# trvon/yams

Hardware: AMD Instinct MI355X
Metric: k-NN QPS + recall@k, 100M x 768 fp32 cosine top-100; ingest GB/s SHA-256+CDC (higher is better)
Workload: dtype i8 (MFMA filter, exact i32 accumulate) + f64 (exact re-score)

## Files before the change

### yams_amd/csrc/scan_i8_kernel.hip

```cpp
#include <cstdlib>
#include <type_traits>

#include "lds_dma.h"
#include "scan_args.h"

namespace yams_accel {

using i32x4v = __attribute__((ext_vector_type(4))) int;

constexpr int I8_ROWS = 256, I8_QUERIES = 256, I8_THREADS = 512;
constexpr int I8_SLAB = 64;
constexpr int I8_NST = 4;
constexpr int I8_A_BYTES = I8_ROWS * I8_SLAB;
constexpr int I8_B_BYTES = I8_QUERIES * I8_SLAB;
constexpr int I8_STAGE = I8_A_BYTES + I8_B_BYTES;
constexpr int I8_BLOCK_ROWS = 64;

__device__ __forceinline__ int i8_swz(int row) {
    const int j = (row >> 2) & 3;
    return (((j ^ (j >> 1)) & 1) << 1) | (j >> 1);
}

__host__ __device__ __forceinline__ uint64_t i8_blocked_offset(uint64_t row, uint32_t col, uint32_t dim) {
    const uint32_t j = static_cast<uint32_t>(row & 15u), slab = col >> 6, chunk = (col >> 4) & 3u;
// ... 1586 lines not shown
    const double per_wave = 8192.0 * p.tau_rank * p.sample_stride / static_cast<double>(p.n_rows ? p.n_rows : 1) * (L.i8_l2 ? 2.0 : 1.0);
    const uint32_t c = static_cast<uint32_t>(per_wave * 4.0 < 8192.0 ? per_wave * 4.0 : 8192.0) + 16;
    return (c + 15) / 16 * 16 < 8192u ? (c + 15) / 16 * 16 : 8192u;
}

hipError_t launch_i8_log_gather(hipStream_t st, const ScanLaunch& L) {
    const uint64_t regions = i8_log_regions(L);
    if (regions == 0) return hipSuccess;
    const ResidentPlan rp = i8_resident_plan(L);
    const I8GatherL2 l2{L.i8_l2_meta, L.i8_row_bias, L.i8_q_bias, L.rows_nsq, L.tau, L.l2_eps};
#ifdef YAMS_ACCEL_MEASURE
    if (rp.use && L.i8_q_form) {
        hipLaunchKernelGGL(i8_log_gather_blocks_kernel, dim3(static_cast<uint32_t>(regions)), dim3(256), 0, st,
                           reinterpret_cast<const int32_t*>(L.log_key), L.log_cnt, L.log_cap, rp.n_qt, L.rows_i8_meta, L.q_meta, L.q_thr,
                           L.plan.n_rows, L.row_mask, L.list_count, L.list, L.plan.list_cap);
        return hipGetLastError();
    }
#endif
    if (rp.use) {
        if (L.i8_l2)
            hipLaunchKernelGGL((i8_log_gather_wave_kernel<true>), dim3(static_cast<uint32_t>(regions)), dim3(256), 0, st,
                               L.log_key, L.log_q, L.log_cnt, L.log_cap, rp.n_qt, L.rows_i8_meta, L.q_meta, L.q_thr, L.list_count,
                               L.list, L.plan.list_cap, l2);
        else
            hipLaunchKernelGGL((i8_log_gather_wave_kernel<false>), dim3(static_cast<uint32_t>(regions)), dim3(256), 0, st,
                               L.log_key, L.log_q, L.log_cnt, L.log_cap, rp.n_qt, L.rows_i8_meta, L.q_meta, L.q_thr, L.list_count,
                               L.list, L.plan.list_cap, l2);
        return hipGetLastError();
    }
    if (L.i8_l2)
        hipLaunchKernelGGL((i8_log_gather_kernel<true>), dim3(static_cast<uint32_t>((regions + 255) / 256)), dim3(256), 0, st,
                           L.log_key, L.log_q, L.log_cnt, L.log_cap, regions, L.rows_i8_meta, L.q_meta, L.q_thr, L.list_count, L.list,
                           L.plan.list_cap, l2);
    else
        hipLaunchKernelGGL((i8_log_gather_kernel<false>), dim3(static_cast<uint32_t>((regions + 255) / 256)), dim3(256), 0, st,
                           L.log_key, L.log_q, L.log_cnt, L.log_cap, regions, L.rows_i8_meta, L.q_meta, L.q_thr, L.list_count, L.list,
                           L.plan.list_cap, l2);
    return hipGetLastError();
}

static bool i8r_direct_rows(uint32_t dim, uint32_t n_qt, bool l2) { (void)dim; return l2 ? n_qt >= 4 : true; }

hipError_t launch_scan_i8(hipStream_t st, const ScanLaunch& L, int mode, int version) {
    (void)version;
    ScanArgs a = make_scan_args(L);
    a.n_sel_tiles = mode == MODE_SAMPLE ? L.plan.n_sample_tiles : L.plan.n_filter_tiles;
    if (a.n_sel_tiles == 0) return hipSuccess;
    const uint32_t hgrid = ((2u * a.n_sel_tiles + 7) / 8) * a.n_qtiles * 8;
    const ResidentPlan rp = i8_resident_plan(L);
    if (mode == MODE_SAMPLE) {
        const uint32_t s_units = (L.plan.n_sample_tiles + 1u) / 2u;
        bool resident_sample = rp.use && !L.i8_l2 && L.i8_sync && L.plan.sample_stride >= 2 && !L.i8_sample_small_grid &&
                               (L.i8_form == 2 ? s_units >= 1u : s_units >= 4u * rp.n_streams);
#ifdef YAMS_ACCEL_MEASURE
        if (const char* sv = std::getenv("YAMS_ACCEL_I8R_SAMPLE")) resident_sample = resident_sample && std::atoi(sv) != 0;
        if (version != 2 && version != 3 && version != 0) resident_sample = false;
#endif
        if (resident_sample) {
            a.i8_sync = L.i8_sync + i8_sync_words(L) / 2u;
            hipLaunchKernelGGL((scan_tiles_i8r_kernel<0, false, true, 0, true>), dim3(rp.grid), dim3(R_THREADS), 0, st, a, s_units, rp.n_qt, rp.n_streams, 1u);
        } else if (L.i8_l2) hipLaunchKernelGGL((scan_tiles_i8h_kernel<MODE_SAMPLE, 0, YAMS_SCAN_L2>), dim3(hgrid), dim3(H_THREADS), 0, st, a);
        else hipLaunchKernelGGL((scan_tiles_i8h_kernel<MODE_SAMPLE>), dim3(hgrid), dim3(H_THREADS), 0, st, a);
        return hipGetLastError();
    }
    bool direct = i8r_direct_rows(L.plan.dim, rp.n_qt, L.i8_l2);
#ifdef YAMS_ACCEL_MEASURE
    if (const char* dv = std::getenv("YAMS_ACCEL_I8R_DIRECT")) direct = std::atoi(dv) != 0;
#endif
    if (L.i8_l2) {
        a.rows_i8_meta = L.i8_l2_meta;
        uint32_t l2_pace_log2 = direct ? 2u : 0u;
#ifdef YAMS_ACCEL_MEASURE
        if (const char* pv = std::getenv("YAMS_ACCEL_I8R_L2_PACE_LOG2")) l2_pace_log2 = static_cast<uint32_t>(std::atoi(pv)) & 31u;
#endif
        const uint32_t l2_window = 1u | (l2_pace_log2 << 16);
        if (rp.use && direct) hipLaunchKernelGGL((scan_tiles_i8r_kernel<0, true, true>), dim3(rp.grid), dim3(R_THREADS), 0, st, a, rp.n_units, rp.n_qt, rp.n_streams, l2_window);
        else if (rp.use) hipLaunchKernelGGL((scan_tiles_i8r_kernel<0, true>), dim3(rp.grid), dim3(R_THREADS), 0, st, a, rp.n_units, rp.n_qt, rp.n_streams, 1u);
        else hipLaunchKernelGGL((scan_tiles_i8h_kernel<MODE_FILTER, 0, YAMS_SCAN_L2>), dim3(hgrid), dim3(H_THREADS), 0, st, a);
        return hipGetLastError();
    }
    uint32_t pace_log2 = direct ? 2u : 0u;
    uint32_t window = 1;
#ifdef YAMS_ACCEL_MEASURE
    if (version >= 41 && version <= 48) {
        if (version == 41) hipLaunchKernelGGL((scan_tiles_i8h_kernel<MODE_FILTER, 1>), dim3(hgrid), dim3(H_THREADS), 0, st, a);
        else if (version == 42) hipLaunchKernelGGL((scan_tiles_i8h_kernel<MODE_FILTER, 2>), dim3(hgrid), dim3(H_THREADS), 0, st, a);
        else if (version == 43) hipLaunchKernelGGL((scan_tiles_i8h_kernel<MODE_FILTER, 3>), dim3(hgrid), dim3(H_THREADS), 0, st, a);
        else if (version == 44) hipLaunchKernelGGL((scan_tiles_i8h_kernel<MODE_FILTER, 4>), dim3(hgrid), dim3(H_THREADS), 0, st, a);
        else if (version == 45) hipLaunchKernelGGL((scan_tiles_i8h_kernel<MODE_FILTER, 5>), dim3(hgrid), dim3(H_THREADS), 0, st, a);
        else if (version == 46) hipLaunchKernelGGL((scan_tiles_i8h_kernel<MODE_FILTER, 6>), dim3(hgrid), dim3(H_THREADS), 0, st, a);
        else if (version == 48) hipLaunchKernelGGL((scan_tiles_i8h_kernel<MODE_FILTER, 8>), dim3(hgrid), dim3(H_THREADS), 0, st, a);
        else hipLaunchKernelGGL((scan_tiles_i8h_kernel<MODE_FILTER, 7>), dim3(hgrid), dim3(H_THREADS), 0, st, a);
        return hipGetLastError();
    }
    if (const char* wv = std::getenv("YAMS_ACCEL_I8R_WINDOW")) window = static_cast<uint32_t>(std::atoi(wv)) & 0xffffu;
    if (const char* pv = std::getenv("YAMS_ACCEL_I8R_PACE_LOG2")) pace_log2 = static_cast<uint32_t>(std::atoi(pv)) & 31u;
    window |= pace_log2 << 16; pace_log2 = 0;
    if (rp.use && version >= 61 && version <= 69) {
        if (version == 61) hipLaunchKernelGGL((scan_tiles_i8r_kernel<1>), dim3(rp.grid), dim3(R_THREADS), 0, st, a, rp.n_units, rp.n_qt, rp.n_streams, window);
        else if (version == 62) hipLaunchKernelGGL((scan_tiles_i8r_kernel<2>), dim3(rp.grid), dim3(R_THREADS), 0, st, a, rp.n_units, rp.n_qt, rp.n_streams, window);
        else if (version == 64) hipLaunchKernelGGL((scan_tiles_i8r_kernel<4>), dim3(rp.grid), dim3(R_THREADS), 0, st, a, rp.n_units, rp.n_qt, rp.n_streams, window);
        else if (version == 68) hipLaunchKernelGGL((scan_tiles_i8r_kernel<8>), dim3(rp.grid), dim3(R_THREADS), 0, st, a, rp.n_units, rp.n_qt, rp.n_streams, window);
        else if (version == 66) hipLaunchKernelGGL((scan_tiles_i8r_kernel<9>), dim3(rp.grid), dim3(R_THREADS), 0, st, a, rp.n_units, rp.n_qt, rp.n_streams, window);
        else if (version == 69) hipLaunchKernelGGL((scan_tiles_i8r_kernel<10, false, true>), dim3(rp.grid), dim3(R_THREADS), 0, st, a, rp.n_units, rp.n_qt, rp.n_streams, window);
        else if (version == 65) hipLaunchKernelGGL((scan_tiles_i8r_kernel<7, false, true>), dim3(rp.grid), dim3(R_THREADS), 0, st, a, rp.n_units, rp.n_qt, rp.n_streams, window);
        else hipLaunchKernelGGL((scan_tiles_i8r_kernel<7>), dim3(rp.grid), dim3(R_THREADS), 0, st, a, rp.n_units, rp.n_qt, rp.n_streams, window);
        return hipGetLastError();
    }
    if (version == 40) {
        hipLaunchKernelGGL((scan_tiles_i8h_kernel<MODE_FILTER>), dim3(hgrid), dim3(H_THREADS), 0, st, a);
        return hipGetLastError();
    }
    if (rp.use && version == 90 && (L.plan.dim == 384 || L.plan.dim == 768)) {
// ... 42 lines not shown
```

### yams_amd/csrc/scan_i8d_kernel.h

```cpp
template <int DUMMY = 0>
__global__ __launch_bounds__(R_THREADS, 1) void scan_tiles_i8d_kernel(ScanArgs a, uint32_t n_units, uint32_t n_qt, uint32_t n_streams, uint32_t window) {
    const uint32_t pace_mask = (1u << ((window >> 16) & 255u)) - 1u;
    __shared__ __attribute__((aligned(16))) unsigned char lds[R_LDS];

    const uint32_t bid = blockIdx.x;
    const uint32_t xcd = bid & 7u, slot = bid >> 3;
    const uint32_t qt = slot % n_qt, st = slot / n_qt;
    if (st >= (n_streams >> 3)) return;
    const uint32_t stream = st * 8u + xcd;
    if (stream >= n_units) return;

#ifdef YAMS_ACCEL_MEASURE
    const uint64_t t_begin = wall_clock64();
#endif
    const int tid = threadIdx.x;
    const int lane = tid & 63;
    const int wid = __builtin_amdgcn_readfirstlane(tid >> 6);
    const int l15 = lane & 15, lq = lane >> 4;
    const uint32_t dim = a.dim;
    const int nslab = dim / I8_SLAB;
    const uint32_t q0 = qt * R_QUERIES;
    const uint32_t lds0 = static_cast<uint32_t>(reinterpret_cast<uintptr_t>((__attribute__((address_space(3))) unsigned char*)lds));
    const uint64_t n_blocks = (a.n_rows + I8_BLOCK_ROWS - 1) / I8_BLOCK_ROWS;
    const uint64_t past_end = n_blocks * I8_BLOCK_ROWS;
    const uint32_t piece_row_stride = static_cast<uint32_t>(nslab) * 1024u;

    struct Geo { uint64_t row0; const unsigned char* base; };
    auto unit_of = [&](uint32_t k) __attribute__((always_inline)) -> uint32_t { return stream + (k >> 1) * n_streams; };
    auto locate = [&](uint32_t k, Geo& g) __attribute__((always_inline)) {
        const uint32_t un_ = unit_of(k);
        const uint32_t sel = un_ < n_units ? 2u * un_ + (k & 1u) : 0xffffffffu;
        uint64_t row0 = past_end;
        if (sel < a.n_sel_tiles) {
            const uint32_t tile = sel + sel / (a.stride - 1u) + 1u;
            row0 = static_cast<uint64_t>(tile) * I8_ROWS + static_cast<uint32_t>((wid & 3) * 64);
        }
        g.row0 = row0;
        const uint64_t rowb = row0 < past_end ? row0 : past_end - 64;
        g.base = reinterpret_cast<const unsigned char*>(a.rows_i8) + (rowb / 16) * piece_row_stride;
    };
    typedef float f2_t __attribute__((ext_vector_type(2)));
    auto meta_ptr = [&](uint64_t row0) __attribute__((always_inline)) -> const float* {
        uint64_t blk = row0 / I8_BLOCK_ROWS;
        if (blk >= n_blocks) blk = n_blocks - 1;
        return a.rows_i8_meta + 2ull * blk;
    };

    {
        const int prow = lane >> 2;
        const int rowB = wid * 16 + prow;
        const uint32_t voffB = static_cast<uint32_t>(rowB) * 64u + ((lane & 3) ^ i8_swz(prow)) * 16u;
        const unsigned char* baseB = reinterpret_cast<const unsigned char*>(a.q_i8) + static_cast<uint64_t>(q0) * 64;
        const uint64_t qslab_bytes = static_cast<uint64_t>(a.q_pad) * 64;
        for (int s = 0; s < nslab; ++s)
            lds_dma16_s(baseB + s * qslab_bytes, voffB, __builtin_amdgcn_readfirstlane(lds0 + s * R_B_SLAB + wid * 1024));
    }
    if (tid < R_QUERIES) reinterpret_cast<f2_t*>(lds + R_ZS_THR)[tid] = reinterpret_cast<const f2_t*>(a.q_thr)[q0 + static_cast<uint32_t>(tid)];
    uint32_t* const pair_cnt = a.i8_sync + (static_cast<uint64_t>(stream) * 4u + static_cast<uint32_t>(wid & 3)) * 32u;
    uint32_t take_v;
    auto take_request = [&]() __attribute__((always_inline)) {
        unsigned long long keep;
        asm volatile("s_mov_b64 %1, exec\n\ts_mov_b64 exec, 1\n\tglobal_atomic_add %0, %2, %3, off sc0\n\ts_mov_b64 exec, %1"
                     : "=&v"(take_v), "=&s"(keep) : "v"(pair_cnt + qt), "v"(1u) : "memory");
    };
    auto take_result = [&]() __attribute__((always_inline)) -> uint32_t {
        asm volatile("" : "+v"(take_v));
        return static_cast<uint32_t>(__builtin_amdgcn_readfirstlane(static_cast<int>(take_v)));
    };
    uint32_t k_cur, k_nxt, k_fut;
    take_request(); asm volatile("s_waitcnt vmcnt(0)" ::: "memory"); k_cur = take_result();
    take_request(); asm volatile("s_waitcnt vmcnt(0)" ::: "memory"); k_nxt = take_result();
    take_request(); asm volatile("s_waitcnt vmcnt(0)" ::: "memory"); k_fut = take_result();
    Geo cur, nxt;
    locate(k_cur, cur);
    float sb, eb;
    {
        const float* mp = meta_ptr(cur.row0);
        const float m0 = mp[0], m1 = mp[1];
        sb = __int_as_float(__builtin_amdgcn_readfirstlane(__float_as_int(m0)));
        eb = __int_as_float(__builtin_amdgcn_readfirstlane(__float_as_int(m1)));
    }
    asm volatile("s_waitcnt vmcnt(0) lgkmcnt(0)" ::: "memory");
    __builtin_amdgcn_s_barrier();

    const int offF = l15 * 64 + ((lq ^ i8_swz(l15)) << 4);
    i32x4v acc[4][8];
    i32x4v fa[3][4], fb[4];
    auto dfetch = [](i32x4v& dst, uint32_t vo, const unsigned char* src) __attribute__((always_inline)) {
        asm volatile("global_load_dwordx4 %0, %1, %2" : "=v"(dst) : "v"(vo), "s"(src) : "memory");
    };
    auto ldq = [&](int slab, int cb) __attribute__((always_inline)) -> i32x4v {
        return *reinterpret_cast<const i32x4v*>(lds + slab * R_B_SLAB + offF + cb * 1024);
    };
#pragma unroll
    for (int rb = 0; rb < 4; ++rb) dfetch(fa[0][rb], static_cast<uint32_t>(offF), cur.base + static_cast<uint32_t>(rb) * piece_row_stride);
#pragma unroll
    for (int rb = 0; rb < 4; ++rb) dfetch(fa[1][rb], static_cast<uint32_t>(offF), cur.base + 1024u + static_cast<uint32_t>(rb) * piece_row_stride);
#pragma unroll
    for (int cb = 0; cb < 3; ++cb) fb[cb] = ldq(0, cb);

    constexpr uint32_t R_POLLS = 1024;
    bool pacing = true;
    const uint32_t R_WINDOW = window & 0xffffu;
    const uint32_t* sync_sib = pair_cnt + (static_cast<uint32_t>(lane) < n_qt ? static_cast<uint32_t>(lane) : qt);
#ifdef YAMS_ACCEL_MEASURE
    uint32_t units_read = 0;
#endif
    uint32_t q_live = 0;
#pragma unroll
    for (int cb = 0; cb < 8; ++cb) q_live |= (q0 + static_cast<uint32_t>(cb * 16 + l15) < a.n_queries) ? 1u << cb : 0u;

    const f2_t* const thr_lds = reinterpret_cast<const f2_t*>(lds + R_ZS_THR) + l15;
    auto acc_init = [&](float sb_, float eb_) __attribute__((always_inline)) {
        const float is = 1.0f / sb_, g = eb_ * is;
#pragma unroll
        for (int cb = 0; cb < 8; ++cb) {
            const f2_t h = thr_lds[cb * 16];
            const int nt = i8_neg_threshold(h[0], is, h[1], g);
#pragma unroll
            for (int rb = 0; rb < 4; ++rb)
#pragma unroll
                for (int r = 0; r < 4; ++r) acc[rb][cb][r] = nt;
        }
    };
    const uint32_t log_region = (stream * n_qt + qt) * 8u + static_cast<uint32_t>(wid);
    const uint64_t region = static_cast<uint64_t>(log_region) * a.log_cap;
    uint32_t log_pos = 0;
    uint64_t* const zs_key = reinterpret_cast<uint64_t*>(lds + R_ZS_LOG + wid * (R_ZS_ENTRIES * 12));
    uint32_t* const zs_q = reinterpret_cast<uint32_t*>(zs_key + R_ZS_ENTRIES);
    uint32_t zs_n = 0;
    auto zs_flush = [&]() __attribute__((always_inline)) {
        for (uint32_t i = static_cast<uint32_t>(__builtin_amdgcn_mbcnt_hi(~0u, __builtin_amdgcn_mbcnt_lo(~0u, 0u))); i < zs_n; i += 64u) {
            const uint64_t key = zs_key[i];
            const uint32_t qi = zs_q[i];
            const uint32_t pos = log_pos + i;
            if (pos < a.log_cap) { a.log_key[region + pos] = key; a.log_q[region + pos] = qi; }
            else atomicOr(&a.q_over[qi], 1u);
        }
        log_pos += zs_n;
        zs_n = 0;
        asm volatile("s_waitcnt vmcnt(0)" ::: "memory");
    };

    acc_init(sb, eb);
    uint32_t sib = 0;
    auto slab = [&](auto j_tag, const unsigned char* a2, int sq, int sqn, auto&& head) __attribute__((always_inline)) {
        constexpr int J = decltype(j_tag)::value;
        constexpr int J2 = (J + 2) % 3;
        asm volatile("s_waitcnt vmcnt(4)" : "+v"(fa[J][0]), "+v"(fa[J][1]), "+v"(fa[J][2]), "+v"(fa[J][3]) :: "memory");
        head();
        __builtin_amdgcn_sched_barrier(0);
#pragma unroll
        for (int c = 0; c < 8; ++c) {
#pragma unroll
            for (int rb = 0; rb < 4; ++rb) {
                asm volatile("v_mfma_i32_16x16x64_i8 %0, %1, %2, %0" : "+v"(acc[rb][c]) : "v"(fa[J][rb]), "v"(fb[c & 3]));
                __builtin_amdgcn_sched_barrier(0);
            }
            if (c < 4) dfetch(fa[J2][c], static_cast<uint32_t>(offF), a2 + static_cast<uint32_t>(c) * piece_row_stride);
            fb[(c + 3) & 3] = c + 3 < 8 ? ldq(sq, c + 3) : ldq(sqn, c + 3 - 8);
            __builtin_amdgcn_sched_barrier(0);
        }
    };
    using J0 = std::integral_constant<int, 0>;
    using J1 = std::integral_constant<int, 1>;
    using J2t = std::integral_constant<int, 2>;

    if (unit_of(k_cur) < n_units) for (;;) {
        const bool more = unit_of(k_nxt) < n_units;
        locate(k_nxt, nxt);
        unsigned long long meta_n;
        {
            const float* mp = meta_ptr(nxt.row0);
            asm volatile("s_load_dwordx2 %0, %1, 0x0" : "=s"(meta_n) : "s"(mp) : "memory");
        }
        const bool pace_now = n_qt > 1 && (k_cur & pace_mask) == 0u;
        auto two_ahead = [&](int s) __attribute__((always_inline)) -> const unsigned char* {
            return s + 2 < nslab ? cur.base + static_cast<uint32_t>(s + 2) * 1024u : nxt.base + static_cast<uint32_t>(s + 2 - nslab) * 1024u;
        };
        asm volatile("s_nop 4" ::: "memory");
        for (int s = 0; s < nslab; s += 3) {
            const bool tail = s + 3 >= nslab;
            slab(J0{}, two_ahead(s), s, s + 1, [] {});
            slab(J1{}, two_ahead(s + 1), s + 1, s + 2, [] {});
            slab(J2t{}, two_ahead(s + 2), s + 2, tail ? 0 : s + 3, [&]() __attribute__((always_inline)) {
                if (tail) {
                    take_request();
                    if (pace_now) asm volatile("global_load_dword %0, %1, off sc0 sc1" : "=v"(sib) : "v"(sync_sib) : "memory");
                }
            });
        }
        asm volatile("s_nop 15\n\ts_nop 7" : "+s"(meta_n));
#ifdef YAMS_ACCEL_MEASURE
        ++units_read;
#endif
        const uint64_t strip = cur.row0;
        uint32_t hot = 0;
#pragma unroll
        for (int cb = 0; cb < 8; ++cb) {
            int m = acc[0][cb][0];
#pragma unroll
            for (int rb = 0; rb < 4; ++rb)
#pragma unroll
                for (int r = 0; r < 4; ++r) m = acc[rb][cb][r] > m ? acc[rb][cb][r] : m;
            if (m >= 0) hot |= 1u << cb;
        }
        hot &= q_live;
        if (strip >= a.n_rows) hot = 0;
        if (__builtin_amdgcn_ballot_w64(hot != 0) != 0) {
            const uint32_t rows_left = strip < a.n_rows ? static_cast<uint32_t>(a.n_rows - strip < 64 ? a.n_rows - strip : 64) : 0u;
            uint32_t base = zs_n;
#pragma unroll
            for (int cb = 0; cb < 8; ++cb) {
                const bool hot_cb = (hot >> cb) & 1u;
                if (__builtin_amdgcn_ballot_w64(hot_cb) == 0) continue;
                const uint32_t qi = q0 + cb * 16 + l15;
                uint32_t pm = 0;
#pragma unroll
                for (int rb = 0; rb < 4; ++rb) {
                    const uint32_t off0 = 16 * rb + 4 * lq;
                    uint32_t mw = 0xfu;
                    if (a.row_mask) { const uint64_t rbase = strip + off0; mw = mask_word(a.row_mask, rbase & ~31ull, a.n_rows) >> (rbase & 31u); }
#pragma unroll
                    for (int r = 0; r < 4; ++r)
                        pm |= (acc[rb][cb][r] >= 0 && off0 + r < rows_left && ((mw >> r) & 1u)) ? 1u << (4 * rb + r) : 0u;
                }
                if (!hot_cb) pm = 0;
                for (;;) {
                    const bool p = pm != 0;
                    const uint64_t m = __builtin_amdgcn_ballot_w64(p);
                    if (m == 0) break;
                    if (base + 64u > static_cast<uint32_t>(R_ZS_ENTRIES)) { zs_n = base; zs_flush(); base = 0; }
                    const int e = p ? __builtin_ctz(pm) : 0;
                    int val = acc[0][cb][0];
#pragma unroll
                    for (int i = 1; i < 16; ++i) val = e == i ? acc[i >> 2][cb][i & 3] : val;
                    const uint32_t pos = base + __builtin_amdgcn_mbcnt_hi(static_cast<uint32_t>(m >> 32), __builtin_amdgcn_mbcnt_lo(static_cast<uint32_t>(m), 0u));
                    base += static_cast<uint32_t>(__builtin_popcountll(m));
                    if (p) {
                        const uint64_t row = strip + static_cast<uint32_t>(16 * (e >> 2) + 4 * lq + (e & 3));
                        zs_key[pos] = (static_cast<uint64_t>(static_cast<uint32_t>(val)) << 32) | static_cast<uint32_t>(row);
                        zs_q[pos] = qi;
                    }
                    pm &= pm - 1u;
                }
            }
            zs_n = base;
        }
        sb = __uint_as_float(static_cast<uint32_t>(meta_n));
        eb = __uint_as_float(static_cast<uint32_t>(meta_n >> 32));
        acc_init(sb, eb);
        __builtin_amdgcn_sched_barrier(0);
        asm volatile("s_waitcnt vmcnt(4)" ::: "memory");
        __builtin_amdgcn_sched_barrier(0);
        const uint32_t k_new = take_result();
        if (more && pacing && pace_now) {
            asm volatile("" : "+v"(sib));
            uint32_t polls = 0;
            for (; polls < R_POLLS; ++polls) {
                if (__builtin_amdgcn_ballot_w64(sib + R_WINDOW < k_new) == 0) break;
                __builtin_amdgcn_s_sleep(8);
                asm volatile("global_load_dword %0, %1, off sc0 sc1\n\ts_waitcnt vmcnt(0)" : "=v"(sib) : "v"(sync_sib) : "memory");
            }
            if (polls == R_POLLS) pacing = false;
        }
        if (!more) break;
        cur = nxt;
        k_cur = k_nxt; k_nxt = k_fut; k_fut = k_new;
    }
    asm volatile("s_waitcnt vmcnt(0)" : "+v"(fa[0][0]), "+v"(fa[0][1]), "+v"(fa[0][2]), "+v"(fa[0][3]), "+v"(fa[1][0]), "+v"(fa[1][1]), "+v"(fa[1][2]),
                 "+v"(fa[1][3]), "+v"(fa[2][0]), "+v"(fa[2][1]), "+v"(fa[2][2]), "+v"(fa[2][3]) :: "memory");
    zs_flush();
    if (__builtin_amdgcn_mbcnt_hi(~0u, __builtin_amdgcn_mbcnt_lo(~0u, 0u)) == 0u) a.log_cnt[log_region] = log_pos < a.log_cap ? log_pos : a.log_cap;
#ifdef YAMS_ACCEL_MEASURE
    if (lane == 0 && n_qt <= 8) {
        uint32_t* const dbg = a.i8_sync + (static_cast<uint64_t>(n_streams) * 4u + static_cast<uint64_t>(stream) * 8u + static_cast<uint32_t>(wid)) * 32u;
        dbg[8 + qt] = static_cast<uint32_t>(t_begin);
        dbg[16 + qt] = static_cast<uint32_t>(wall_clock64());
        dbg[24 + qt] = units_read;
    }
#endif
}
```

Baseline: 17100.

## Add deep-pipelined i8 sample kernel for dims 384/768 sharing the i8d body

Moves the i8d resident kernel body into a shared include parameterized by a SAMPLE flag and instantiates a sample-mode variant (scan_tiles_i8ds_kernel). For dims 384 and 768 the resident sample pass now uses this three-stage prefetched MFMA pipeline in place of the generic i8r sample kernel. The sample variant computes per-group float maxima via the query metadata and writes them to gmax, and it skips the threshold setup and pacing. This is meant to overlap row loads with MFMA work during sampling, at the cost of a second large kernel instantiation and a separate code path to keep correct.

```diff
diff --git a/yams_amd/csrc/scan_i8_kernel.hip b/yams_amd/csrc/scan_i8_kernel.hip
--- a/yams_amd/csrc/scan_i8_kernel.hip
+++ b/yams_amd/csrc/scan_i8_kernel.hip
@@ -1662,13 +1662,15 @@
         const uint32_t s_units = (L.plan.n_sample_tiles + 1u) / 2u;
         bool resident_sample = rp.use && !L.i8_l2 && L.i8_sync && L.plan.sample_stride >= 2 && !L.i8_sample_small_grid &&
                                (L.i8_form == 2 ? s_units >= 1u : s_units >= 4u * rp.n_streams);
+        bool deep_sample = L.plan.dim == 384 || L.plan.dim == 768;
 #ifdef YAMS_ACCEL_MEASURE
-        if (const char* sv = std::getenv("YAMS_ACCEL_I8R_SAMPLE")) resident_sample = resident_sample && std::atoi(sv) != 0;
+        if (const char* sv = std::getenv("YAMS_ACCEL_I8R_SAMPLE")) { resident_sample = resident_sample && std::atoi(sv) != 0; deep_sample = deep_sample && std::atoi(sv) != 2; }
         if (version != 2 && version != 3 && version != 0) resident_sample = false;
 #endif
         if (resident_sample) {
             a.i8_sync = L.i8_sync + i8_sync_words(L) / 2u;
-            hipLaunchKernelGGL((scan_tiles_i8r_kernel<0, false, true, 0, true>), dim3(rp.grid), dim3(R_THREADS), 0, st, a, s_units, rp.n_qt, rp.n_streams, 1u);
+            if (deep_sample) hipLaunchKernelGGL((scan_tiles_i8ds_kernel<0>), dim3(rp.grid), dim3(R_THREADS), 0, st, a, s_units, rp.n_qt, rp.n_streams, 1u);
+            else hipLaunchKernelGGL((scan_tiles_i8r_kernel<0, false, true, 0, true>), dim3(rp.grid), dim3(R_THREADS), 0, st, a, s_units, rp.n_qt, rp.n_streams, 1u);
         } else if (L.i8_l2) hipLaunchKernelGGL((scan_tiles_i8h_kernel<MODE_SAMPLE, 0, YAMS_SCAN_L2>), dim3(hgrid), dim3(H_THREADS), 0, st, a);
         else hipLaunchKernelGGL((scan_tiles_i8h_kernel<MODE_SAMPLE>), dim3(hgrid), dim3(H_THREADS), 0, st, a);
         return hipGetLastError();
diff --git a/yams_amd/csrc/scan_i8d_body.h b/yams_amd/csrc/scan_i8d_body.h
--- /dev/null
+++ b/yams_amd/csrc/scan_i8d_body.h
@@ -0,0 +1,338 @@
+    const uint32_t pace_mask = (1u << ((window >> 16) & 255u)) - 1u;
+    __shared__ __attribute__((aligned(16))) unsigned char lds[R_LDS];
+
+    const uint32_t bid = blockIdx.x;
+    const uint32_t xcd = bid & 7u, slot = bid >> 3;
+    const uint32_t qt = slot % n_qt, st = slot / n_qt;
+    if (st >= (n_streams >> 3)) return;
+    const uint32_t stream = st * 8u + xcd;
+    if (stream >= n_units) return;
+
+#ifdef YAMS_ACCEL_MEASURE
+    const uint64_t t_begin = wall_clock64();
+#endif
+    const int tid = threadIdx.x;
+    const int lane = tid & 63;
+    const int wid = __builtin_amdgcn_readfirstlane(tid >> 6);
+    const int l15 = lane & 15, lq = lane >> 4;
+    const uint32_t dim = a.dim;
+    const int nslab = dim / I8_SLAB;
+    const uint32_t q0 = qt * R_QUERIES;
+    const uint32_t lds0 = static_cast<uint32_t>(reinterpret_cast<uintptr_t>((__attribute__((address_space(3))) unsigned char*)lds));
+    const uint64_t n_blocks = (a.n_rows + I8_BLOCK_ROWS - 1) / I8_BLOCK_ROWS;
+    const uint64_t past_end = n_blocks * I8_BLOCK_ROWS;
+    const uint32_t piece_row_stride = static_cast<uint32_t>(nslab) * 1024u;
+
+    struct Geo { uint64_t row0; const unsigned char* base; };
+    auto unit_of = [&](uint32_t k) __attribute__((always_inline)) -> uint32_t { return stream + (k >> 1) * n_streams; };
+    auto locate = [&](uint32_t k, Geo& g) __attribute__((always_inline)) {
+        const uint32_t un_ = unit_of(k);
+        const uint32_t sel = un_ < n_units ? 2u * un_ + (k & 1u) : 0xffffffffu;
+        uint64_t row0 = past_end;
+        if (sel < a.n_sel_tiles) {
+            const uint32_t tile = SAMPLE ? sel * a.stride : sel + sel / (a.stride - 1u) + 1u;
+            row0 = static_cast<uint64_t>(tile) * I8_ROWS + static_cast<uint32_t>((wid & 3) * 64);
+        }
+        g.row0 = row0;
+        const uint64_t rowb = row0 < past_end ? row0 : past_end - 64;
+        g.base = reinterpret_cast<const unsigned char*>(a.rows_i8) + (rowb / 16) * piece_row_stride;
+    };
+    typedef float f2_t __attribute__((ext_vector_type(2)));
+    auto meta_ptr = [&](uint64_t row0) __attribute__((always_inline)) -> const float* {
+        uint64_t blk = row0 / I8_BLOCK_ROWS;
+        if (blk >= n_blocks) blk = n_blocks - 1;
+        return a.rows_i8_meta + 2ull * blk;
+    };
+
+    {
+        const int prow = lane >> 2;
+        const int rowB = wid * 16 + prow;
+        const uint32_t voffB = static_cast<uint32_t>(rowB) * 64u + ((lane & 3) ^ i8_swz(prow)) * 16u;
+        const unsigned char* baseB = reinterpret_cast<const unsigned char*>(a.q_i8) + static_cast<uint64_t>(q0) * 64;
+        const uint64_t qslab_bytes = static_cast<uint64_t>(a.q_pad) * 64;
+        for (int s = 0; s < nslab; ++s)
+            lds_dma16_s(baseB + s * qslab_bytes, voffB, __builtin_amdgcn_readfirstlane(lds0 + s * R_B_SLAB + wid * 1024));
+    }
+    if (SAMPLE) {
+        if (tid < R_QUERIES) reinterpret_cast<float4*>(lds + R_ZS_THR)[tid] = reinterpret_cast<const float4*>(a.q_meta)[q0 + static_cast<uint32_t>(tid)];
+    } else if (tid < R_QUERIES) reinterpret_cast<f2_t*>(lds + R_ZS_THR)[tid] = reinterpret_cast<const f2_t*>(a.q_thr)[q0 + static_cast<uint32_t>(tid)];
+    uint32_t* const pair_cnt = a.i8_sync + (static_cast<uint64_t>(stream) * 4u + static_cast<uint32_t>(wid & 3)) * 32u;
+    uint32_t take_v;
+    auto take_request = [&]() __attribute__((always_inline)) {
+        unsigned long long keep;
+        asm volatile("s_mov_b64 %1, exec\n\ts_mov_b64 exec, 1\n\tglobal_atomic_add %0, %2, %3, off sc0\n\ts_mov_b64 exec, %1"
+                     : "=&v"(take_v), "=&s"(keep) : "v"(pair_cnt + qt), "v"(1u) : "memory");
+    };
+    auto take_result = [&]() __attribute__((always_inline)) -> uint32_t {
+        asm volatile("" : "+v"(take_v));
+        return static_cast<uint32_t>(__builtin_amdgcn_readfirstlane(static_cast<int>(take_v)));
+    };
+    uint32_t k_cur, k_nxt, k_fut;
+    take_request(); asm volatile("s_waitcnt vmcnt(0)" ::: "memory"); k_cur = take_result();
+    take_request(); asm volatile("s_waitcnt vmcnt(0)" ::: "memory"); k_nxt = take_result();
+    take_request(); asm volatile("s_waitcnt vmcnt(0)" ::: "memory"); k_fut = take_result();
+    Geo cur, nxt;
+    locate(k_cur, cur);
+    float sb, eb;
+    {
+        const float* mp = meta_ptr(cur.row0);
+        const float m0 = mp[0], m1 = mp[1];
+        sb = __int_as_float(__builtin_amdgcn_readfirstlane(__float_as_int(m0)));
+        eb = __int_as_float(__builtin_amdgcn_readfirstlane(__float_as_int(m1)));
+    }
+    if (SAMPLE) asm volatile("" :: "s"(sb), "s"(eb));
+    asm volatile("s_waitcnt vmcnt(0) lgkmcnt(0)" ::: "memory");
+    __builtin_amdgcn_s_barrier();
+
+    const int offF = l15 * 64 + ((lq ^ i8_swz(l15)) << 4);
+    i32x4v acc[4][8];
+    i32x4v fa[3][4], fb[4];
+    auto dfetch = [](i32x4v& dst, uint32_t vo, const unsigned char* src) __attribute__((always_inline)) {
+        asm volatile("global_load_dwordx4 %0, %1, %2" : "=v"(dst) : "v"(vo), "s"(src) : "memory");
+    };
+    auto ldq = [&](int slab, int cb) __attribute__((always_inline)) -> i32x4v {
+        return *reinterpret_cast<const i32x4v*>(lds + slab * R_B_SLAB + offF + cb * 1024);
+    };
+#pragma unroll
+    for (int rb = 0; rb < 4; ++rb) dfetch(fa[0][rb], static_cast<uint32_t>(offF), cur.base + static_cast<uint32_t>(rb) * piece_row_stride);
+#pragma unroll
+    for (int rb = 0; rb < 4; ++rb) dfetch(fa[1][rb], static_cast<uint32_t>(offF), cur.base + 1024u + static_cast<uint32_t>(rb) * piece_row_stride);
+#pragma unroll
+    for (int cb = 0; cb < 3; ++cb) fb[cb] = ldq(0, cb);
+    if (SAMPLE) asm volatile("s_waitcnt vmcnt(4)" : "+v"(fa[0][0]), "+v"(fa[0][1]), "+v"(fa[0][2]), "+v"(fa[0][3]) :: "memory");
+
+    constexpr uint32_t R_POLLS = 1024;
+    bool pacing = true;
+    const uint32_t R_WINDOW = window & 0xffffu;
+    const uint32_t* sync_sib = pair_cnt + (static_cast<uint32_t>(lane) < n_qt ? static_cast<uint32_t>(lane) : qt);
+#ifdef YAMS_ACCEL_MEASURE
+    uint32_t units_read = 0;
+#endif
+    uint32_t q_live = 0;
+#pragma unroll
+    for (int cb = 0; cb < 8; ++cb) q_live |= (q0 + static_cast<uint32_t>(cb * 16 + l15) < a.n_queries) ? 1u << cb : 0u;
+
+    const f2_t* const thr_lds = reinterpret_cast<const f2_t*>(lds + R_ZS_THR) + l15;
+    auto acc_init = [&](float sb_, float eb_) __attribute__((always_inline)) {
+        const float is = 1.0f / sb_, g = eb_ * is;
+#pragma unroll
+        for (int cb = 0; cb < 8; ++cb) {
+            int nt = 0;
+            if (!SAMPLE) {
+                const f2_t h = thr_lds[cb * 16];
+                nt = i8_neg_threshold(h[0], is, h[1], g);
+            }
+#pragma unroll
+            for (int rb = 0; rb < 4; ++rb)
+#pragma unroll
+                for (int r = 0; r < 4; ++r) acc[rb][cb][r] = nt;
+        }
+    };
+    const uint32_t log_region = (stream * n_qt + qt) * 8u + static_cast<uint32_t>(wid);
+    const uint64_t region = static_cast<uint64_t>(log_region) * a.log_cap;
+    uint32_t log_pos = 0;
+    uint64_t* const zs_key = reinterpret_cast<uint64_t*>(lds + R_ZS_LOG + wid * (R_ZS_ENTRIES * 12));
+    uint32_t* const zs_q = reinterpret_cast<uint32_t*>(zs_key + R_ZS_ENTRIES);
+    uint32_t zs_n = 0;
+    auto zs_flush = [&]() __attribute__((always_inline)) {
+        for (uint32_t i = static_cast<uint32_t>(__builtin_amdgcn_mbcnt_hi(~0u, __builtin_amdgcn_mbcnt_lo(~0u, 0u))); i < zs_n; i += 64u) {
+            const uint64_t key = zs_key[i];
+            const uint32_t qi = zs_q[i];
+            const uint32_t pos = log_pos + i;
+            if (pos < a.log_cap) { a.log_key[region + pos] = key; a.log_q[region + pos] = qi; }
+            else atomicOr(&a.q_over[qi], 1u);
+        }
+        log_pos += zs_n;
+        zs_n = 0;
+        asm volatile("s_waitcnt vmcnt(0)" ::: "memory");
+    };
+
+    acc_init(sb, eb);
+    uint32_t sib = 0;
+    auto slab = [&](auto j_tag, const unsigned char* a2, int sq, int sqn, auto&& head, bool landed = false) __attribute__((always_inline)) {
+        constexpr int J = decltype(j_tag)::value;
+        constexpr int J2 = (J + 2) % 3;
+        if (!landed) asm volatile("s_waitcnt vmcnt(4)" : "+v"(fa[J][0]), "+v"(fa[J][1]), "+v"(fa[J][2]), "+v"(fa[J][3]) :: "memory");
+        head();
+        __builtin_amdgcn_sched_barrier(0);
+#pragma unroll
+        for (int c = 0; c < 8; ++c) {
+#pragma unroll
+            for (int rb = 0; rb < 4; ++rb) {
+                asm volatile("v_mfma_i32_16x16x64_i8 %0, %1, %2, %0" : "+v"(acc[rb][c]) : "v"(fa[J][rb]), "v"(fb[c & 3]));
+                __builtin_amdgcn_sched_barrier(0);
+            }
+            if (c < 4) dfetch(fa[J2][c], static_cast<uint32_t>(offF), a2 + static_cast<uint32_t>(c) * piece_row_stride);
+            fb[(c + 3) & 3] = c + 3 < 8 ? ldq(sq, c + 3) : ldq(sqn, c + 3 - 8);
+            __builtin_amdgcn_sched_barrier(0);
+        }
+    };
+    using J0 = std::integral_constant<int, 0>;
+    using J1 = std::integral_constant<int, 1>;
+    using J2t = std::integral_constant<int, 2>;
+
+    if (unit_of(k_cur) < n_units) for (;;) {
+        const bool more = unit_of(k_nxt) < n_units;
+        locate(k_nxt, nxt);
+        unsigned long long meta_n;
+        {
+            const float* mp = meta_ptr(nxt.row0);
+            asm volatile("s_load_dwordx2 %0, %1, 0x0" : "=s"(meta_n) : "s"(mp) : "memory");
+        }
+        const bool pace_now = !SAMPLE && n_qt > 1 && (k_cur & pace_mask) == 0u;
+        auto two_ahead = [&](int s) __attribute__((always_inline)) -> const unsigned char* {
+            return s + 2 < nslab ? cur.base + static_cast<uint32_t>(s + 2) * 1024u : nxt.base + static_cast<uint32_t>(s + 2 - nslab) * 1024u;
+        };
+        asm volatile("s_nop 4" ::: "memory");
+        for (int s = 0; s < nslab; s += 3) {
+            const bool tail = s + 3 >= nslab;
+            slab(J0{}, two_ahead(s), s, s + 1, [] {}, SAMPLE && s == 0);
+            slab(J1{}, two_ahead(s + 1), s + 1, s + 2, [] {});
+            slab(J2t{}, two_ahead(s + 2), s + 2, tail ? 0 : s + 3, [&]() __attribute__((always_inline)) {
+                if (tail) {
+                    take_request();
+                    if (pace_now) asm volatile("global_load_dword %0, %1, off sc0 sc1" : "=v"(sib) : "v"(sync_sib) : "memory");
+                }
+            });
+        }
+        asm volatile("s_nop 15\n\ts_nop 7" : "+s"(meta_n));
+#ifdef YAMS_ACCEL_MEASURE
+        ++units_read;
+#endif
+        const uint64_t strip = cur.row0;
+        uint32_t k_new;
+        if (SAMPLE) {
+            const uint32_t sel_c = 2u * unit_of(k_cur) + (k_cur & 1u);
+            const bool live = sel_c < a.n_sel_tiles;
+            uint32_t ord[8];
+#pragma unroll
+            for (int cb = 0; cb < 8; ++cb) ord[cb] = 0u;
+            if (live) {
+                const float ninf = -__builtin_inff();
+                uint32_t mw[4];
+#pragma unroll
+                for (int rb = 0; rb < 4; ++rb) {
+                    const uint64_t rbase = strip + static_cast<uint32_t>(16 * rb + 4 * lq);
+                    mw[rb] = a.row_mask ? mask_word(a.row_mask, rbase & ~31ull, a.n_rows) >> (rbase & 31u) : 0xfu;
+                }
+#pragma unroll
+                for (int cb = 0; cb < 8; ++cb) {
+                    const float4 qm = reinterpret_cast<const float4*>(lds + R_ZS_THR)[cb * 16 + l15];
+                    const float S = sb * qm.x, K = fmaf(eb, qm.y, qm.z);
+                    float m = ninf;
+#pragma unroll
+                    for (int rb = 0; rb < 4; ++rb) {
+                        const uint64_t rbase = strip + static_cast<uint32_t>(16 * rb + 4 * lq);
+#pragma unroll
+                        for (int r = 0; r < 4; ++r) {
+                            const float uu = fmaf(static_cast<float>(acc[rb][cb][r]), S, K);
+                            m = fmaxf(m, (rbase + r < a.n_rows && ((mw[rb] >> r) & 1u)) ? uu : ninf);
+                        }
+                    }
+                    ord[cb] = (m != m) ? 0xffffffffu : f2ord(m);
+                }
+            }
+            sb = __uint_as_float(static_cast<uint32_t>(meta_n));
+            eb = __uint_as_float(static_cast<uint32_t>(meta_n >> 32));
+            acc_init(sb, eb);
+            __builtin_amdgcn_sched_barrier(0);
+            asm volatile("s_waitcnt vmcnt(4)" : "+v"(ord[0]), "+v"(ord[1]), "+v"(ord[2]), "+v"(ord[3]), "+v"(ord[4]), "+v"(ord[5]), "+v"(ord[6]), "+v"(ord[7]) :: "memory");
+            __builtin_amdgcn_sched_barrier(0);
+            k_new = take_result();
+            if (live) {
+                const uint32_t gid = (sel_c * static_cast<uint32_t>(I8_ROWS) + static_cast<uint32_t>((wid & 3) * 64)) / 16u + static_cast<uint32_t>(lq);
+#pragma unroll
+                for (int cb = 0; cb < 8; ++cb) {
+                    const uint32_t qi = q0 + static_cast<uint32_t>(cb * 16 + l15);
+                    if (qi < a.n_queries) a.gmax[static_cast<uint64_t>(qi) * a.n_groups + gid] = ord[cb];
+                }
+            }
+        } else {
+        uint32_t hot = 0;
+#pragma unroll
+        for (int cb = 0; cb < 8; ++cb) {
+            int m = acc[0][cb][0];
+#pragma unroll
+            for (int rb = 0; rb < 4; ++rb)
+#pragma unroll
+                for (int r = 0; r < 4; ++r) m = acc[rb][cb][r] > m ? acc[rb][cb][r] : m;
+            if (m >= 0) hot |= 1u << cb;
+        }
+        hot &= q_live;
+        if (strip >= a.n_rows) hot = 0;
+        if (__builtin_amdgcn_ballot_w64(hot != 0) != 0) {
+            const uint32_t rows_left = strip < a.n_rows ? static_cast<uint32_t>(a.n_rows - strip < 64 ? a.n_rows - strip : 64) : 0u;
+            uint32_t base = zs_n;
+#pragma unroll
+            for (int cb = 0; cb < 8; ++cb) {
+                const bool hot_cb = (hot >> cb) & 1u;
+                if (__builtin_amdgcn_ballot_w64(hot_cb) == 0) continue;
+                const uint32_t qi = q0 + cb * 16 + l15;
+                uint32_t pm = 0;
+#pragma unroll
+                for (int rb = 0; rb < 4; ++rb) {
+                    const uint32_t off0 = 16 * rb + 4 * lq;
+                    uint32_t mw = 0xfu;
+                    if (a.row_mask) { const uint64_t rbase = strip + off0; mw = mask_word(a.row_mask, rbase & ~31ull, a.n_rows) >> (rbase & 31u); }
+#pragma unroll
+                    for (int r = 0; r < 4; ++r)
+                        pm |= (acc[rb][cb][r] >= 0 && off0 + r < rows_left && ((mw >> r) & 1u)) ? 1u << (4 * rb + r) : 0u;
+                }
+                if (!hot_cb) pm = 0;
+                for (;;) {
+                    const bool p = pm != 0;
+                    const uint64_t m = __builtin_amdgcn_ballot_w64(p);
+                    if (m == 0) break;
+                    if (base + 64u > static_cast<uint32_t>(R_ZS_ENTRIES)) { zs_n = base; zs_flush(); base = 0; }
+                    const int e = p ? __builtin_ctz(pm) : 0;
+                    int val = acc[0][cb][0];
+#pragma unroll
+                    for (int i = 1; i < 16; ++i) val = e == i ? acc[i >> 2][cb][i & 3] : val;
+                    const uint32_t pos = base + __builtin_amdgcn_mbcnt_hi(static_cast<uint32_t>(m >> 32), __builtin_amdgcn_mbcnt_lo(static_cast<uint32_t>(m), 0u));
+                    base += static_cast<uint32_t>(__builtin_popcountll(m));
+                    if (p) {
+                        const uint64_t row = strip + static_cast<uint32_t>(16 * (e >> 2) + 4 * lq + (e & 3));
+                        zs_key[pos] = (static_cast<uint64_t>(static_cast<uint32_t>(val)) << 32) | static_cast<uint32_t>(row);
+                        zs_q[pos] = qi;
+                    }
+                    pm &= pm - 1u;
+                }
+            }
+            zs_n = base;
+        }
+        sb = __uint_as_float(static_cast<uint32_t>(meta_n));
+        eb = __uint_as_float(static_cast<uint32_t>(meta_n >> 32));
+        acc_init(sb, eb);
+        __builtin_amdgcn_sched_barrier(0);
+        asm volatile("s_waitcnt vmcnt(4)" ::: "memory");
+        __builtin_amdgcn_sched_barrier(0);
+        k_new = take_result();
+        if (more && pacing && pace_now) {
+            asm volatile("" : "+v"(sib));
+            uint32_t polls = 0;
+            for (; polls < R_POLLS; ++polls) {
+                if (__builtin_amdgcn_ballot_w64(sib + R_WINDOW < k_new) == 0) break;
+                __builtin_amdgcn_s_sleep(8);
+                asm volatile("global_load_dword %0, %1, off sc0 sc1\n\ts_waitcnt vmcnt(0)" : "=v"(sib) : "v"(sync_sib) : "memory");
+            }
+            if (polls == R_POLLS) pacing = false;
+        }
+        }
+        if (!more) break;
+        cur = nxt;
+        k_cur = k_nxt; k_nxt = k_fut; k_fut = k_new;
+    }
+    asm volatile("s_waitcnt vmcnt(0)" : "+v"(fa[0][0]), "+v"(fa[0][1]), "+v"(fa[0][2]), "+v"(fa[0][3]), "+v"(fa[1][0]), "+v"(fa[1][1]), "+v"(fa[1][2]),
+                 "+v"(fa[1][3]), "+v"(fa[2][0]), "+v"(fa[2][1]), "+v"(fa[2][2]), "+v"(fa[2][3]) :: "memory");
+    if (!SAMPLE) {
+        zs_flush();
+        if (__builtin_amdgcn_mbcnt_hi(~0u, __builtin_amdgcn_mbcnt_lo(~0u, 0u)) == 0u) a.log_cnt[log_region] = log_pos < a.log_cap ? log_pos : a.log_cap;
+    }
+#ifdef YAMS_ACCEL_MEASURE
+    if (lane == 0 && n_qt <= 8) {
+        uint32_t* const dbg = a.i8_sync + (static_cast<uint64_t>(n_streams) * 4u + static_cast<uint64_t>(stream) * 8u + static_cast<uint32_t>(wid)) * 32u;
+        dbg[8 + qt] = static_cast<uint32_t>(t_begin);
+        dbg[16 + qt] = static_cast<uint32_t>(wall_clock64());
+        dbg[24 + qt] = units_read;
+    }
+#endif
diff --git a/yams_amd/csrc/scan_i8d_kernel.h b/yams_amd/csrc/scan_i8d_kernel.h
--- a/yams_amd/csrc/scan_i8d_kernel.h
+++ b/yams_amd/csrc/scan_i8d_kernel.h
@@ -1,283 +1,12 @@
+
 template <int DUMMY = 0>
 __global__ __launch_bounds__(R_THREADS, 1) void scan_tiles_i8d_kernel(ScanArgs a, uint32_t n_units, uint32_t n_qt, uint32_t n_streams, uint32_t window) {
-    const uint32_t pace_mask = (1u << ((window >> 16) & 255u)) - 1u;
-    __shared__ __attribute__((aligned(16))) unsigned char lds[R_LDS];
+    constexpr bool SAMPLE = false;
+#include "scan_i8d_body.h"
+}
 
-    const uint32_t bid = blockIdx.x;
-    const uint32_t xcd = bid & 7u, slot = bid >> 3;
-    const uint32_t qt = slot % n_qt, st = slot / n_qt;
-    if (st >= (n_streams >> 3)) return;
-    const uint32_t stream = st * 8u + xcd;
-    if (stream >= n_units) return;
-
-#ifdef YAMS_ACCEL_MEASURE
-    const uint64_t t_begin = wall_clock64();
-#endif
-    const int tid = threadIdx.x;
-    const int lane = tid & 63;
-    const int wid = __builtin_amdgcn_readfirstlane(tid >> 6);
-    const int l15 = lane & 15, lq = lane >> 4;
-    const uint32_t dim = a.dim;
-    const int nslab = dim / I8_SLAB;
-    const uint32_t q0 = qt * R_QUERIES;
-    const uint32_t lds0 = static_cast<uint32_t>(reinterpret_cast<uintptr_t>((__attribute__((address_space(3))) unsigned char*)lds));
-    const uint64_t n_blocks = (a.n_rows + I8_BLOCK_ROWS - 1) / I8_BLOCK_ROWS;
-    const uint64_t past_end = n_blocks * I8_BLOCK_ROWS;
-    const uint32_t piece_row_stride = static_cast<uint32_t>(nslab) * 1024u;
-
-    struct Geo { uint64_t row0; const unsigned char* base; };
-    auto unit_of = [&](uint32_t k) __attribute__((always_inline)) -> uint32_t { return stream + (k >> 1) * n_streams; };
-    auto locate = [&](uint32_t k, Geo& g) __attribute__((always_inline)) {
-        const uint32_t un_ = unit_of(k);
-        const uint32_t sel = un_ < n_units ? 2u * un_ + (k & 1u) : 0xffffffffu;
-        uint64_t row0 = past_end;
-        if (sel < a.n_sel_tiles) {
-            const uint32_t tile = sel + sel / (a.stride - 1u) + 1u;
-            row0 = static_cast<uint64_t>(tile) * I8_ROWS + static_cast<uint32_t>((wid & 3) * 64);
-        }
-        g.row0 = row0;
-        const uint64_t rowb = row0 < past_end ? row0 : past_end - 64;
-        g.base = reinterpret_cast<const unsigned char*>(a.rows_i8) + (rowb / 16) * piece_row_stride;
-    };
-    typedef float f2_t __attribute__((ext_vector_type(2)));
-    auto meta_ptr = [&](uint64_t row0) __attribute__((always_inline)) -> const float* {
-        uint64_t blk = row0 / I8_BLOCK_ROWS;
-        if (blk >= n_blocks) blk = n_blocks - 1;
-        return a.rows_i8_meta + 2ull * blk;
-    };
-
-    {
-        const int prow = lane >> 2;
-        const int rowB = wid * 16 + prow;
-        const uint32_t voffB = static_cast<uint32_t>(rowB) * 64u + ((lane & 3) ^ i8_swz(prow)) * 16u;
-        const unsigned char* baseB = reinterpret_cast<const unsigned char*>(a.q_i8) + static_cast<uint64_t>(q0) * 64;
-        const uint64_t qslab_bytes = static_cast<uint64_t>(a.q_pad) * 64;
-        for (int s = 0; s < nslab; ++s)
-            lds_dma16_s(baseB + s * qslab_bytes, voffB, __builtin_amdgcn_readfirstlane(lds0 + s * R_B_SLAB + wid * 1024));
-    }
-    if (tid < R_QUERIES) reinterpret_cast<f2_t*>(lds + R_ZS_THR)[tid] = reinterpret_cast<const f2_t*>(a.q_thr)[q0 + static_cast<uint32_t>(tid)];
-    uint32_t* const pair_cnt = a.i8_sync + (static_cast<uint64_t>(stream) * 4u + static_cast<uint32_t>(wid & 3)) * 32u;
-    uint32_t take_v;
-    auto take_request = [&]() __attribute__((always_inline)) {
-        unsigned long long keep;
-        asm volatile("s_mov_b64 %1, exec\n\ts_mov_b64 exec, 1\n\tglobal_atomic_add %0, %2, %3, off sc0\n\ts_mov_b64 exec, %1"
-                     : "=&v"(take_v), "=&s"(keep) : "v"(pair_cnt + qt), "v"(1u) : "memory");
-    };
-    auto take_result = [&]() __attribute__((always_inline)) -> uint32_t {
-        asm volatile("" : "+v"(take_v));
-        return static_cast<uint32_t>(__builtin_amdgcn_readfirstlane(static_cast<int>(take_v)));
-    };
-    uint32_t k_cur, k_nxt, k_fut;
-    take_request(); asm volatile("s_waitcnt vmcnt(0)" ::: "memory"); k_cur = take_result();
-    take_request(); asm volatile("s_waitcnt vmcnt(0)" ::: "memory"); k_nxt = take_result();
-    take_request(); asm volatile("s_waitcnt vmcnt(0)" ::: "memory"); k_fut = take_result();
-    Geo cur, nxt;
-    locate(k_cur, cur);
-    float sb, eb;
-    {
-        const float* mp = meta_ptr(cur.row0);
-        const float m0 = mp[0], m1 = mp[1];
-        sb = __int_as_float(__builtin_amdgcn_readfirstlane(__float_as_int(m0)));
-        eb = __int_as_float(__builtin_amdgcn_readfirstlane(__float_as_int(m1)));
-    }
-    asm volatile("s_waitcnt vmcnt(0) lgkmcnt(0)" ::: "memory");
-    __builtin_amdgcn_s_barrier();
-
-    const int offF = l15 * 64 + ((lq ^ i8_swz(l15)) << 4);
-    i32x4v acc[4][8];
-    i32x4v fa[3][4], fb[4];
-    auto dfetch = [](i32x4v& dst, uint32_t vo, const unsigned char* src) __attribute__((always_inline)) {
-        asm volatile("global_load_dwordx4 %0, %1, %2" : "=v"(dst) : "v"(vo), "s"(src) : "memory");
-    };
-    auto ldq = [&](int slab, int cb) __attribute__((always_inline)) -> i32x4v {
-        return *reinterpret_cast<const i32x4v*>(lds + slab * R_B_SLAB + offF + cb * 1024);
-    };
-#pragma unroll
-    for (int rb = 0; rb < 4; ++rb) dfetch(fa[0][rb], static_cast<uint32_t>(offF), cur.base + static_cast<uint32_t>(rb) * piece_row_stride);
-#pragma unroll
-    for (int rb = 0; rb < 4; ++rb) dfetch(fa[1][rb], static_cast<uint32_t>(offF), cur.base + 1024u + static_cast<uint32_t>(rb) * piece_row_stride);
-#pragma unroll
-    for (int cb = 0; cb < 3; ++cb) fb[cb] = ldq(0, cb);
-
-    constexpr uint32_t R_POLLS = 1024;
-    bool pacing = true;
-    const uint32_t R_WINDOW = window & 0xffffu;
-    const uint32_t* sync_sib = pair_cnt + (static_cast<uint32_t>(lane) < n_qt ? static_cast<uint32_t>(lane) : qt);
-#ifdef YAMS_ACCEL_MEASURE
-    uint32_t units_read = 0;
-#endif
-    uint32_t q_live = 0;
-#pragma unroll
-    for (int cb = 0; cb < 8; ++cb) q_live |= (q0 + static_cast<uint32_t>(cb * 16 + l15) < a.n_queries) ? 1u << cb : 0u;
-
-    const f2_t* const thr_lds = reinterpret_cast<const f2_t*>(lds + R_ZS_THR) + l15;
-    auto acc_init = [&](float sb_, float eb_) __attribute__((always_inline)) {
-        const float is = 1.0f / sb_, g = eb_ * is;
-#pragma unroll
-        for (int cb = 0; cb < 8; ++cb) {
-            const f2_t h = thr_lds[cb * 16];
-            const int nt = i8_neg_threshold(h[0], is, h[1], g);
-#pragma unroll
-            for (int rb = 0; rb < 4; ++rb)
-#pragma unroll
-                for (int r = 0; r < 4; ++r) acc[rb][cb][r] = nt;
-        }
-    };
-    const uint32_t log_region = (stream * n_qt + qt) * 8u + static_cast<uint32_t>(wid);
-    const uint64_t region = static_cast<uint64_t>(log_region) * a.log_cap;
-    uint32_t log_pos = 0;
-    uint64_t* const zs_key = reinterpret_cast<uint64_t*>(lds + R_ZS_LOG + wid * (R_ZS_ENTRIES * 12));
-    uint32_t* const zs_q = reinterpret_cast<uint32_t*>(zs_key + R_ZS_ENTRIES);
-    uint32_t zs_n = 0;
-    auto zs_flush = [&]() __attribute__((always_inline)) {
-        for (uint32_t i = static_cast<uint32_t>(__builtin_amdgcn_mbcnt_hi(~0u, __builtin_amdgcn_mbcnt_lo(~0u, 0u))); i < zs_n; i += 64u) {
-            const uint64_t key = zs_key[i];
-            const uint32_t qi = zs_q[i];
-            const uint32_t pos = log_pos + i;
-            if (pos < a.log_cap) { a.log_key[region + pos] = key; a.log_q[region + pos] = qi; }
-            else atomicOr(&a.q_over[qi], 1u);
-        }
-        log_pos += zs_n;
-        zs_n = 0;
-        asm volatile("s_waitcnt vmcnt(0)" ::: "memory");
-    };
-
-    acc_init(sb, eb);
-    uint32_t sib = 0;
-    auto slab = [&](auto j_tag, const unsigned char* a2, int sq, int sqn, auto&& head) __attribute__((always_inline)) {
-        constexpr int J = decltype(j_tag)::value;
-        constexpr int J2 = (J + 2) % 3;
-        asm volatile("s_waitcnt vmcnt(4)" : "+v"(fa[J][0]), "+v"(fa[J][1]), "+v"(fa[J][2]), "+v"(fa[J][3]) :: "memory");
-        head();
-        __builtin_amdgcn_sched_barrier(0);
-#pragma unroll
-        for (int c = 0; c < 8; ++c) {
-#pragma unroll
-            for (int rb = 0; rb < 4; ++rb) {
-                asm volatile("v_mfma_i32_16x16x64_i8 %0, %1, %2, %0" : "+v"(acc[rb][c]) : "v"(fa[J][rb]), "v"(fb[c & 3]));
-                __builtin_amdgcn_sched_barrier(0);
-            }
-            if (c < 4) dfetch(fa[J2][c], static_cast<uint32_t>(offF), a2 + static_cast<uint32_t>(c) * piece_row_stride);
-            fb[(c + 3) & 3] = c + 3 < 8 ? ldq(sq, c + 3) : ldq(sqn, c + 3 - 8);
-            __builtin_amdgcn_sched_barrier(0);
-        }
-    };
-    using J0 = std::integral_constant<int, 0>;
-    using J1 = std::integral_constant<int, 1>;
-    using J2t = std::integral_constant<int, 2>;
-
-    if (unit_of(k_cur) < n_units) for (;;) {
-        const bool more = unit_of(k_nxt) < n_units;
-        locate(k_nxt, nxt);
-        unsigned long long meta_n;
-        {
-            const float* mp = meta_ptr(nxt.row0);
-            asm volatile("s_load_dwordx2 %0, %1, 0x0" : "=s"(meta_n) : "s"(mp) : "memory");
-        }
-        const bool pace_now = n_qt > 1 && (k_cur & pace_mask) == 0u;
-        auto two_ahead = [&](int s) __attribute__((always_inline)) -> const unsigned char* {
-            return s + 2 < nslab ? cur.base + static_cast<uint32_t>(s + 2) * 1024u : nxt.base + static_cast<uint32_t>(s + 2 - nslab) * 1024u;
-        };
-        asm volatile("s_nop 4" ::: "memory");
-        for (int s = 0; s < nslab; s += 3) {
-            const bool tail = s + 3 >= nslab;
-            slab(J0{}, two_ahead(s), s, s + 1, [] {});
-            slab(J1{}, two_ahead(s + 1), s + 1, s + 2, [] {});
-            slab(J2t{}, two_ahead(s + 2), s + 2, tail ? 0 : s + 3, [&]() __attribute__((always_inline)) {
-                if (tail) {
-                    take_request();
-                    if (pace_now) asm volatile("global_load_dword %0, %1, off sc0 sc1" : "=v"(sib) : "v"(sync_sib) : "memory");
-                }
-            });
-        }
-        asm volatile("s_nop 15\n\ts_nop 7" : "+s"(meta_n));
-#ifdef YAMS_ACCEL_MEASURE
-        ++units_read;
-#endif
-        const uint64_t strip = cur.row0;
-        uint32_t hot = 0;
-#pragma unroll
-        for (int cb = 0; cb < 8; ++cb) {
-            int m = acc[0][cb][0];
-#pragma unroll
-            for (int rb = 0; rb < 4; ++rb)
-#pragma unroll
-                for (int r = 0; r < 4; ++r) m = acc[rb][cb][r] > m ? acc[rb][cb][r] : m;
-            if (m >= 0) hot |= 1u << cb;
-        }
-        hot &= q_live;
-        if (strip >= a.n_rows) hot = 0;
-        if (__builtin_amdgcn_ballot_w64(hot != 0) != 0) {
-            const uint32_t rows_left = strip < a.n_rows ? static_cast<uint32_t>(a.n_rows - strip < 64 ? a.n_rows - strip : 64) : 0u;
-            uint32_t base = zs_n;
-#pragma unroll
-            for (int cb = 0; cb < 8; ++cb) {
-                const bool hot_cb = (hot >> cb) & 1u;
-                if (__builtin_amdgcn_ballot_w64(hot_cb) == 0) continue;
-                const uint32_t qi = q0 + cb * 16 + l15;
-                uint32_t pm = 0;
-#pragma unroll
-                for (int rb = 0; rb < 4; ++rb) {
-                    const uint32_t off0 = 16 * rb + 4 * lq;
-                    uint32_t mw = 0xfu;
-                    if (a.row_mask) { const uint64_t rbase = strip + off0; mw = mask_word(a.row_mask, rbase & ~31ull, a.n_rows) >> (rbase & 31u); }
-#pragma unroll
-                    for (int r = 0; r < 4; ++r)
-                        pm |= (acc[rb][cb][r] >= 0 && off0 + r < rows_left && ((mw >> r) & 1u)) ? 1u << (4 * rb + r) : 0u;
-                }
-                if (!hot_cb) pm = 0;
-                for (;;) {
-                    const bool p = pm != 0;
-                    const uint64_t m = __builtin_amdgcn_ballot_w64(p);
-                    if (m == 0) break;
-                    if (base + 64u > static_cast<uint32_t>(R_ZS_ENTRIES)) { zs_n = base; zs_flush(); base = 0; }
-                    const int e = p ? __builtin_ctz(pm) : 0;
-                    int val = acc[0][cb][0];
-#pragma unroll
-                    for (int i = 1; i < 16; ++i) val = e == i ? acc[i >> 2][cb][i & 3] : val;
-                    const uint32_t pos = base + __builtin_amdgcn_mbcnt_hi(static_cast<uint32_t>(m >> 32), __builtin_amdgcn_mbcnt_lo(static_cast<uint32_t>(m), 0u));
-                    base += static_cast<uint32_t>(__builtin_popcountll(m));
-                    if (p) {
-                        const uint64_t row = strip + static_cast<uint32_t>(16 * (e >> 2) + 4 * lq + (e & 3));
-                        zs_key[pos] = (static_cast<uint64_t>(static_cast<uint32_t>(val)) << 32) | static_cast<uint32_t>(row);
-                        zs_q[pos] = qi;
-                    }
-                    pm &= pm - 1u;
-                }
-            }
-            zs_n = base;
-        }
-        sb = __uint_as_float(static_cast<uint32_t>(meta_n));
-        eb = __uint_as_float(static_cast<uint32_t>(meta_n >> 32));
-        acc_init(sb, eb);
-        __builtin_amdgcn_sched_barrier(0);
-        asm volatile("s_waitcnt vmcnt(4)" ::: "memory");
-        __builtin_amdgcn_sched_barrier(0);
-        const uint32_t k_new = take_result();
-        if (more && pacing && pace_now) {
-            asm volatile("" : "+v"(sib));
-            uint32_t polls = 0;
-            for (; polls < R_POLLS; ++polls) {
-                if (__builtin_amdgcn_ballot_w64(sib + R_WINDOW < k_new) == 0) break;
-                __builtin_amdgcn_s_sleep(8);
-                asm volatile("global_load_dword %0, %1, off sc0 sc1\n\ts_waitcnt vmcnt(0)" : "=v"(sib) : "v"(sync_sib) : "memory");
-            }
-            if (polls == R_POLLS) pacing = false;
-        }
-        if (!more) break;
-        cur = nxt;
-        k_cur = k_nxt; k_nxt = k_fut; k_fut = k_new;
-    }
-    asm volatile("s_waitcnt vmcnt(0)" : "+v"(fa[0][0]), "+v"(fa[0][1]), "+v"(fa[0][2]), "+v"(fa[0][3]), "+v"(fa[1][0]), "+v"(fa[1][1]), "+v"(fa[1][2]),
-                 "+v"(fa[1][3]), "+v"(fa[2][0]), "+v"(fa[2][1]), "+v"(fa[2][2]), "+v"(fa[2][3]) :: "memory");
-    zs_flush();
-    if (__builtin_amdgcn_mbcnt_hi(~0u, __builtin_amdgcn_mbcnt_lo(~0u, 0u)) == 0u) a.log_cnt[log_region] = log_pos < a.log_cap ? log_pos : a.log_cap;
-#ifdef YAMS_ACCEL_MEASURE
-    if (lane == 0 && n_qt <= 8) {
-        uint32_t* const dbg = a.i8_sync + (static_cast<uint64_t>(n_streams) * 4u + static_cast<uint64_t>(stream) * 8u + static_cast<uint32_t>(wid)) * 32u;
-        dbg[8 + qt] = static_cast<uint32_t>(t_begin);
-        dbg[16 + qt] = static_cast<uint32_t>(wall_clock64());
-        dbg[24 + qt] = units_read;
-    }
-#endif
+template <int DUMMY = 0>
+__global__ __launch_bounds__(R_THREADS, 1) void scan_tiles_i8ds_kernel(ScanArgs a, uint32_t n_units, uint32_t n_qt, uint32_t n_streams, uint32_t window) {
+    constexpr bool SAMPLE = true;
+#include "scan_i8d_body.h"
 }
```

Result: no change. 17190, median of 5 (+0.5%).
